# sjtuyinjie/Ground-Fusion2

Measured on AMD Instinct MI355X. Metric: sliding-window solves/sec (10-kf, 2k landmarks), higher is better.
Workload: dtype f64; 1 GPU; BASELINE configs[1]: 10-keyframe VI-wheel window, 2000 landmarks (K=9457 visual factors avg), marginalisation prior n=86, full optimization() = <=8 dogleg iterations + re-anchor + MARGIN_OLD; windows_per_gpu=8192, unique_windows=8, parallelism=windows sharded over 1 rank(s), no collective

## Files before the change

### ground-fusion2_amd/csrc/gfbe_devutil.h

```cpp
#pragma once
#include "gfbe_device.h"

namespace gfd {

#define GF_MIN_DIAG 1e-6
#define GF_MAX_DIAG 1e32
#define GF_MIN_MU 1e-8
#define GF_MAX_MU 1.0
#define GF_MU_INC 10.0

__device__ __forceinline__ double wave_sum(double v) {
#pragma unroll
  for (int o = 32; o > 0; o >>= 1) v += __shfl_down(v, o, 64);
  return v;
}
__device__ __forceinline__ double wave_max(double v) {
#pragma unroll
  for (int o = 32; o > 0; o >>= 1) v = fmax(v, __shfl_down(v, o, 64));
  return v;
}
__device__ __forceinline__ double block_sum(double v, double *scratch ) {
  v = wave_sum(v);
  const int lane = threadIdx.x & 63, wid = threadIdx.x >> 6;
  __syncthreads();
  if (lane == 0) scratch[wid] = v;
  __syncthreads();
  double r = 0.0;
  if (threadIdx.x == 0) for (int i = 0; i < (int)((blockDim.x + 63) >> 6); i++) r += scratch[i];
  return r;
}
__device__ __forceinline__ double block_max(double v, double *scratch) {
  v = wave_max(v);
  const int lane = threadIdx.x & 63, wid = threadIdx.x >> 6;
  __syncthreads();
  if (lane == 0) scratch[wid] = v;
  __syncthreads();
  double r = 0.0;
  if (threadIdx.x == 0) for (int i = 0; i < (int)((blockDim.x + 63) >> 6); i++) r = fmax(r, scratch[i]);
  return r;
}

template <int NQ>
__device__ __forceinline__ void block_reduce_multi(const double (&v)[NQ], unsigned maxmask, double *scratch, int tid = -1) {
  if (tid < 0) tid = threadIdx.x;
  const int lane = tid & 63, wid = tid >> 6, nw = (blockDim.x + 63) >> 6;
  __syncthreads();
#pragma unroll
  for (int q = 0; q < NQ; q++) {
    const double r = ((maxmask >> q) & 1) ? wave_max(v[q]) : wave_sum(v[q]);
    if (lane == 0) scratch[q * 16 + wid] = r;
  }
  __syncthreads();
  if (tid < NQ) {
// ... 43 lines not shown
```

### ground-fusion2_amd/csrc/gfbe_kernels.hip

```cpp
#include "gfbe_devutil.h"
#include "gfbe_factors.h"
#include "gfbe_gnss_item.h"
#include <type_traits>

namespace gfd {

#ifndef GFBE_ASM_U
#define GFBE_ASM_U 4
#endif
#if GFBE_DIAG
#define ASM_TP_ON(d) (!(d).asm_legacy)
#else
#define ASM_TP_ON(d) true
#endif
#ifndef GFBE_KVIS_WAVES
#define GFBE_KVIS_WAVES 3
#endif
#ifndef GFBE_KVIS_STAMP
#define GFBE_KVIS_STAMP 0
#endif

#define PREP_WSYNC() do { __threadfence_block(); __builtin_amdgcn_wave_barrier(); } while (0)
template <int n>
__device__ __forceinline__ int sqrt_info_from_cov_wave(const double *cov, double *lu, double *inv, double *U, const int lane) {
// ... 208 lines not shown
  const WinDesc &ds = d.desc[w];
  if (tile >= ds.n_tiles || !TILE_OWNED(d, tile)) return;
  const WinCtl &c = d.ctl[w];
  if (MODE == 0 && !SPEC && (c.done || c.reuse)) return;
  if (CAND && (c.done || !c.have_step)) return;
  int sframe = 0;
#pragma unroll
  for (int q = 1; q < NF; q++) sframe += (tile >= ds.sf_tile_begin[q]) ? 1 : 0;
  if (MODE == 2 && sframe != 0) return;
  const int buf = CAND ? 1 - c.cur : c.cur;
  const double *X = (MODE == 2) ? d.xout + (size_t)w * NA : d.x + ((size_t)w * 2 + buf) * NA;
  const double *lamv = d.lam + (size_t)buf * d.tot_lm;

#if GFBE_KVIS_STAMP
  double *kstamp = d.timing + (size_t)d.B * 32;
  const bool kst = MODE == 0 && w == d.B / 2 && tile == 0 && threadIdx.x == 0 && c.iter == 0;
#define KSTAMP(i) do { if (kst) kstamp[i] = (double)wall_clock64(); } while (0)
#else
#define KSTAMP(i) do { } while (0)
#endif
#if GFBE_LIN_STAMP
  unsigned long long *lst = (unsigned long long *)(d.timing + (size_t)d.B * 32);
  const bool lstamp = KS > 1 && MODE == 0 && tile == 0 && (threadIdx.x & 63) == 0 && (WS || threadIdx.x == 0);
#define LSTAMP(i) do { if (lstamp && kq == 0) lst[i] = wall_clock64(); } while (0)
#define LSTAMP_ANY(i) do { if (lstamp) lst[i] = wall_clock64(); } while (0)
#else
#define LSTAMP(i) do { } while (0)
#define LSTAMP_ANY(i) do { } while (0)
#endif
  LSTAMP(14);
  KSTAMP(0);
  constexpr bool YM = (MODE == 0 && !FULL);
  typedef typename std::conditional<FULL, PairConst, typename std::conditional<MODE == 2, PairConstR, PairConstY>::type>::type PCT;
  constexpr int PCW = (MODE == 1) ? 12 : sizeof(PCT) / sizeof(double), XLD = FULL ? XS_LD : 17;
  __shared__ PCT pcs[NF];
  __shared__ FrameConst fcs;
  __shared__ double xs_own[(MODE == 1 || WS) ? 1 : LM_TILE * XLD];
  double *const xs = WS ? wsm + (size_t)kq * (LM_TILE * XLD) : xs_own;
  const int lane = WS ? (threadIdx.x & 63) : threadIdx.x;
  const int slot = ds.lm_off + tile * LM_TILE + lane;
  const size_t TL = d.tot_lm;
  const bool tdc = YM || (MODE == 1 && !d.vis_full);
  const int nobq = tdc ? 2 : 5;
  const int info = d.lm_info[slot];
  const double pix = d.lm_pts[0 * TL + slot], piy = d.lm_pts[1 * TL + slot], piz = d.lm_pts[2 * TL + slot];
  double vix = 0.0, viy = 0.0, tdi = 0.0;
  if (!tdc) { vix = d.lm_pts[3 * TL + slot]; viy = d.lm_pts[4 * TL + slot]; tdi = d.lm_pts[5 * TL + slot]; }
  const bool chead = CAND && head;
  double lam = chead ? d.lam[(size_t)c.cur * TL + slot] : lamv[slot];
  double c_sl = 0.0, c_vl = 0.0, c_yl = 0.0;
  if (chead) { c_sl = d.lm_sl[slot]; c_vl = d.lm_vl[slot]; c_yl = d.lm_yl[slot]; }
  const double td = X[A_TD];
  double nob[5] = {0.0, 0.0, 0.0, 0.0, 0.0};
  {
    const double *ob = d.lm_obs + (size_t)kq * 5 * TL + slot;
#pragma unroll
    for (int q = 0; q < 5; q++) if (q < nobq) nob[q] = ob[q * TL];
  }
  constexpr int NLATER = KS > 1 ? (MAXOBS + KS - 1) / KS - 1 : 0;
  double nobl[NLATER > 0 ? NLATER : 1][5];
#pragma unroll
  for (int u = 0; u < NLATER; u++) {
#pragma unroll
    for (int q = 0; q < 5; q++) nobl[u][q] = 0.0;
    if (kq + (u + 1) * KS < MAXOBS) {
      const double *ob = d.lm_obs + (size_t)(kq + (u + 1) * KS) * 5 * TL + slot;
#pragma unroll
      for (int q = 0; q < 5; q++) if (q < nobq) nobl[u][q] = ob[q * TL];
    }
  }
// ... 33 lines not shown
  }
  if (chead) {
    double d2, n2;
    lam = candidate_lm(lam, c_sl, c_vl, c_yl, c.c1, c.c2, valid && !is_const && m > 0, d2, n2);
    d.lam[(size_t)(1 - c.cur) * TL + slot] = lam;
    d2 = wave_sum(d2); n2 = wave_sum(n2);
    if (lane == 0) {
      double *o = d.tile_cand + ((size_t)w * d.max_tiles + tile) * 4;
      o[1] = d2; o[2] = n2;
    }
  }

  constexpr int NHC = FULL ? HC : 6;
  double hC[NHC], Hll = 0.0, gl = 0.0;
#pragma unroll
  for (int q = 0; q < NHC; q++) hC[q] = 0.0;
  if (MODE != 1 && !FULL && !YM) {
    double *xr = xs + lane * XLD;
    xr[13] = 0.0; xr[14] = 0.0; xr[15] = 0.0;
  }
  double ycx = 0.0, ycy = 0.0, ycz = 0.0, yinv_l = 0.0, Dsum[3] = {0.0, 0.0, 0.0};
  vec3 yf = mk3(0.0, 0.0, 0.0), ye = yf, yx = yf;
  if (YM || MODE == 1) {
    const double dti = tdc ? 0.0 : td - tdi;
    yinv_l = 1.0 / lam;
    ycx = (tdc ? pix : __builtin_fma(-dti, vix, pix)) * yinv_l; ycy = (tdc ? piy : __builtin_fma(-dti, viy, piy)) * yinv_l; ycz = piz * yinv_l;
    if (YM) {
#pragma unroll
      for (int a = 0; a < 3; a++) {
        yf[a] = __builtin_fma(fcs.W(a, 0), ycx, __builtin_fma(fcs.W(a, 1), ycy, fcs.W(a, 2) * ycz));
        ye[a] = yf[a] + fcs.wt[a];
        yx[a] = ye[a] + fcs.dPc[a];
      }
      double *xr = xs + lane * XLD;
      xr[7] = 0.0; xr[15] = 0.0;
    }
  }
  KSTAMP(2);
  double *contrib = KS > 1 ? d.vis_contrib + (((size_t)w * d.max_tiles + tile) * MAXOBS) * (VC_STRIDE * LM_TILE) + lane : nullptr;
  for (int k = kq; k < mmax; k += KS) {
    if (k < 5) KSTAMP(3 + 5 * k);
    double r[2], Ji[12], Jj[12], Je[FULL ? 12 : 1], Jl[2], Jt[2], hp[6];
    const double pjx = nob[0], pjy = nob[1], vjx = nob[2], vjy = nob[3], tdj = nob[4];
    if (KS > 1) {
#pragma unroll
      for (int q = 0; q < 5; q++) nob[q] = nobl[0][q];
#pragma unroll
      for (int u = 0; u + 1 < NLATER; u++) {
#pragma unroll
        for (int q = 0; q < 5; q++) nobl[u][q] = nobl[u + 1][q];
      }
    } else if (k + KS < mmax) {
      const double *ob = d.lm_obs + (size_t)(k + KS) * 5 * TL + slot;
#pragma unroll
      for (int q = 0; q < 5; q++) if (q < nobq) nob[q] = ob[q * TL];
    }
    if constexpr (YM) {
      double *xr = xs + lane * XLD;
      if (k < m) {
        const PCT &pc = pcs[sframe + 1 + k];
        double g0[3], g1[3];
        const double ck = visual_lin_y(pc, ycx, ycy, ycz, yf, yinv_l, td, pjx, pjy, vjx, vjy, tdj, sq, delta, r, g0, g1, Jl);
        if (KS > 1) contrib[((size_t)k * VC_STRIDE + 15) * LM_TILE] = ck; else cost += ck;
        const vec3 y0 = cross3(mk3(g0[0], g0[1], g0[2]), yx), y1 = cross3(mk3(g1[0], g1[1], g1[2]), yx);
        const double w0 = is_const ? 0.0 : Jl[0], w1 = is_const ? 0.0 : Jl[1];
        vec3 dv;
#pragma unroll
        for (int q = 0; q < 3; q++) dv[q] = __builtin_fma(g0[q], w0, g1[q] * w1);
        if (KS > 1) {
          double *cb = contrib + (size_t)k * VC_STRIDE * LM_TILE;
          cb[0] = __builtin_fma(w0, w0, w1 * w1);
          cb[LM_TILE] = __builtin_fma(w0, r[0], w1 * r[1]);
#pragma unroll
          for (int q = 0; q < 3; q++) cb[(2 + q) * LM_TILE] = dv[q];
        } else {
          Hll += __builtin_fma(w0, w0, w1 * w1);
          gl += __builtin_fma(w0, r[0], w1 * r[1]);
#pragma unroll
          for (int q = 0; q < 3; q++) Dsum[q] += dv[q];
        }
#pragma unroll
        for (int q = 0; q < 3; q++) hp[q] = dv[q];
#pragma unroll
        for (int q = 0; q < 3; q++) { xr[q] = g0[q]; xr[3 + q] = y0[q]; xr[8 + q] = g1[q]; xr[11 + q] = y1[q]; }
        xr[6] = r[0]; xr[14] = r[1];
      } else {
#pragma unroll
        for (int q = 0; q < 7; q++) { xr[q] = 0.0; xr[8 + q] = 0.0; }
      }
#pragma unroll
      for (int q = 0; q < 2; q++) asm volatile("" : "+v"(nob[q]));
      if (k < m) {
#pragma unroll
        for (int q = 0; q < 3; q++) d.lm_hP[((size_t)k * 6 + q) * TL + slot] = hp[q];
      }
      typedef double dbl4_y __attribute__((ext_vector_type(4)));
      dbl4_y acc0 = {0, 0, 0, 0};
      const int lr = lane & 15, lk = lane >> 4;
      __threadfence_block();
      __builtin_amdgcn_wave_barrier();
#pragma unroll
      for (int blk = 0; blk < LM_TILE / 4 / 8; blk++) {
        double va[8];
#pragma unroll
        for (int u = 0; u < 8; u++) va[u] = xs[(4 * (8 * blk + u) + lk) * XLD + lr];
#pragma unroll
        for (int u = 0; u < 8; u++) acc0 = __builtin_amdgcn_mfma_f64_16x16x4f64(va[u], va[u], acc0, 0, 0, 0);
      }
      __builtin_amdgcn_wave_barrier();
      const double s0 = acc0[0] + __shfl_down(acc0[2], 8, 64), s1 = acc0[1] + __shfl_down(acc0[3], 8, 64);
      double *vo = d.vis_part + (((size_t)w * d.max_tiles + tile) * MAXOBS + k) * VPY_STRIDE;
      if (lr < 7) {
        { const int a = lk; if (a <= lr) vo[7 * a - a * (a - 1) / 2 + lr - a] = s0; }
        { const int a = lk + 4; if (a <= lr) vo[7 * a - a * (a - 1) / 2 + lr - a] = s1; }
      }
      __builtin_amdgcn_wave_barrier();
    }
    if constexpr (MODE == 1) {
      if (k < m) cost += visual_cost_y(pcs[sframe + 1 + k], ycx, ycy, ycz, td, pjx, pjy, vjx, vjy, tdj, sq, delta);
    }
    if constexpr (!YM && MODE != 1) {
    if (k < m) {
      const double ck = visual_lin<MODE != 1, FULL>(pcs[sframe + 1 + k], lam, td, pix, piy, piz, pjx, pjy, vix, viy, vjx, vjy, tdi, tdj,
                                                    sq, delta, r, Ji, Jj, Je, Jl, Jt);
      if (KS > 1) contrib[((size_t)k * VC_STRIDE + 15) * LM_TILE] = ck; else cost += ck;
      if (MODE != 1) {
        if (FULL && write_records) {
          double *rb = d.rec + ((size_t)ds.rec_off + d.lm_rec[(size_t)k * TL + slot]) * REC;
          rb[0] = r[0]; rb[1] = r[1];
#pragma unroll
          for (int q = 0; q < 6; q++) {
            rb[2 + q] = Ji[q]; rb[8 + q] = Jj[q]; rb[14 + q] = Je[FULL ? q : 0];
            rb[22 + q] = Ji[6 + q]; rb[28 + q] = Jj[6 + q]; rb[34 + q] = Je[FULL ? 6 + q : 0];
          }
          rb[20] = Jl[0]; rb[21] = Jt[0]; rb[40] = Jl[1]; rb[41] = Jt[1];
        }
        const double w0 = (is_const && MODE == 0) ? 0.0 : Jl[0], w1 = (is_const && MODE == 0) ? 0.0 : Jl[1];
        if (KS > 1) {
          double *cb = contrib + (size_t)k * VC_STRIDE * LM_TILE;
          cb[0] = __builtin_fma(w0, w0, w1 * w1);
          cb[LM_TILE] = __builtin_fma(w0, r[0], w1 * r[1]);
#pragma unroll
          for (int q = 0; q < 6; q++) {
            cb[(2 + q) * LM_TILE] = __builtin_fma(Ji[q], w0, Ji[6 + q] * w1);
            if (FULL) cb[(8 + q) * LM_TILE] = __builtin_fma(Je[q], w0, Je[6 + q] * w1);
            hp[q] = __builtin_fma(Jj[q], w0, Jj[6 + q] * w1);
          }
          if (FULL) cb[14 * LM_TILE] = __builtin_fma(Jt[0], w0, Jt[1] * w1);
        } else {
// ... 182 lines not shown
}

__device__ __forceinline__ double candidate_tile(const BatchDev &d, const WinDesc &ds, const WinCtl &c, const int w, const int tile, const int t);
template <int MODE, bool FULL, bool SPEC = false>
__global__ __launch_bounds__(LM_TILE, (MODE == 0 && !FULL) ? GFBE_KVIS_WAVES : 2) void k_vis(BatchDev d0, int write_records) {
  const BatchDev d = MODE == 0 ? lin_view(d0, SPEC ? 1 - d0.ctl[blockIdx.x].lb : d0.ctl[blockIdx.x].lb) : d0;
  vis_body<MODE, FULL, 1, SPEC>(d, (MODE == 1 || SPEC) ? 0 : write_records, blockIdx.x, blockIdx.y, 0, (MODE == 1 || SPEC) && write_records);
}

#ifndef VIS_CHUNK
#define VIS_CHUNK 4
#endif
template <bool SPEC>
__global__ __launch_bounds__(LM_TILE, GFBE_KVIS_WAVES) void k_vis_chunk(BatchDev d0, int head_in, int nsub) {
  const int w = blockIdx.x;
  const WinCtl &c = d0.ctl[w];
  if (!SPEC && (c.done || c.reuse)) return;
  if (SPEC && (c.done || !c.have_step)) return;
  const int lbw = SPEC ? 1 - c.lb : c.lb;
  const BatchDev d = lin_view(d0, lbw);
  const WinDesc &ds = d.desc[w];
  const int sframe = blockIdx.y / nsub, sub = blockIdx.y - sframe * nsub;
  const int t0 = ds.sf_tile_begin[sframe] + VIS_CHUNK * sub, t1 = min(t0 + VIS_CHUNK, ds.sf_tile_begin[sframe + 1]);
  if (t0 >= t1) return;
  const int cur = c.cur, buf = SPEC ? 1 - cur : cur;
  const double *X = d.x + ((size_t)w * 2 + buf) * NA;
  const bool chead = SPEC && head_in;
  const double c1 = c.c1, c2 = c.c2;
  const bool first = !SPEC && c.iter == 0;
  const double mu_w = SPEC ? mu_after_accept(c.mu) : c.mu;
  const double sq = d.opt.vis_sqrt_info, delta = d.opt.huber_delta;
  const int jac_scale = d.opt.jacobi_scaling;
  const int lm_off_c = ds.lm_off;
  constexpr int XLD = 17;
  __shared__ PairConstY pcs[NF];
  __shared__ FrameConst fcs;
  __shared__ double xs[LM_TILE * XLD];
  const int lane = threadIdx.x;
  const size_t TL = d.tot_lm;
  int p_info;
  double p_pt[3], p_lam, p_sl = 0.0, p_vl = 0.0, p_yl = 0.0, p_ob[2];
#define VC_PREFETCH(TILE)                                                                                           \
  {                                                                                                                  \
    const int slot_ = lm_off_c + (TILE) * LM_TILE + lane;                                                            \
    p_info = d.lm_info[slot_];                                                                                       \
    _Pragma("unroll") for (int q = 0; q < 3; q++) p_pt[q] = d.lm_pts[(size_t)q * TL + slot_];                        \
    p_lam = d.lam[(size_t)(chead ? cur : buf) * TL + slot_];                                                         \
    if (chead) { p_sl = d.lm_sl[slot_]; p_vl = d.lm_vl[slot_]; p_yl = d.lm_yl[slot_]; }                              \
    p_ob[0] = d.lm_obs[slot_]; p_ob[1] = d.lm_obs[TL + slot_];                                                       \
  }
  VC_PREFETCH(t0)
  const double td = X[A_TD];
  {
    const double *src = d.pc + (((size_t)w * 3 + buf) * NPAIR + sframe * NF) * PC_DOUBLES;
    static_assert(PCY_DOUBLES <= LM_TILE && FC_DOUBLES <= LM_TILE, "one lane per entry of a pair record");
    const int ql = min(lane, (int)PCY_DOUBLES - 1);
    double rec[NF - 1];
#pragma unroll
    for (int jj = 0; jj < NF - 1; jj++) rec[jj] = src[(size_t)min(sframe + 1 + jj, NF - 1) * PC_DOUBLES + ql];
    const double fcv = src[(size_t)sframe * PC_DOUBLES + min(lane, (int)FC_DOUBLES - 1)];
#pragma unroll
    for (int jj = 0; jj < NF - 1; jj++) if (sframe + 1 + jj < NF && lane < (int)PCY_DOUBLES) ((double *)&pcs[min(sframe + 1 + jj, NF - 1)])[lane] = rec[jj];
    if (lane < (int)FC_DOUBLES) ((double *)&fcs)[lane] = fcv;
  }
  __syncthreads();
  for (int tile = t0; tile < t1; tile++) {
    const int slot = lm_off_c + tile * LM_TILE + lane;
    const int info = p_info;
    const double pix = p_pt[0], piy = p_pt[1], piz = p_pt[2];
    double lam = p_lam;
    const double c_sl = p_sl, c_vl = p_vl, c_yl = p_yl;
    double nob[2] = {p_ob[0], p_ob[1]};
    if (tile + 1 < t1) VC_PREFETCH(tile + 1)
    const bool valid = (info >> 24) & 1;
    const int m = valid ? ((info >> 8) & 0xff) : 0;
    const bool is_const = (info >> 16) & 1;
    int mmax = m;
#pragma unroll
    for (int o = 32; o > 0; o >>= 1) mmax = max(mmax, __shfl_xor(mmax, o, 64));
    double cost = 0.0;
    if (chead) {
      double d2, n2;
      lam = candidate_lm(lam, c_sl, c_vl, c_yl, c1, c2, valid && !is_const && m > 0, d2, n2);
      d.lam[(size_t)(1 - cur) * TL + slot] = lam;
      d2 = wave_sum(d2); n2 = wave_sum(n2);
      if (lane == 0) {
        double *o = d.tile_cand + ((size_t)w * d.max_tiles + tile) * 4;
        o[1] = d2; o[2] = n2;
      }
    }
    double Hll = 0.0, gl = 0.0, Dsum[3] = {0.0, 0.0, 0.0};
    const double yinv_l = 1.0 / lam;
    const double ycx = pix * yinv_l, ycy = piy * yinv_l, ycz = piz * yinv_l;
    vec3 yf, ye, yx;
#pragma unroll
    for (int a = 0; a < 3; a++) {
      yf[a] = __builtin_fma(fcs.W(a, 0), ycx, __builtin_fma(fcs.W(a, 1), ycy, fcs.W(a, 2) * ycz));
      ye[a] = yf[a] + fcs.wt[a];
      yx[a] = ye[a] + fcs.dPc[a];
    }
    double *xr = xs + lane * XLD;
    xr[7] = 0.0; xr[15] = 0.0;
    for (int k = 0; k < mmax; k++) {
      double r[2], Jl[2], hp[3];
      const double pjx = nob[0], pjy = nob[1];
      if (k + 1 < mmax) {
        const double *ob = d.lm_obs + (size_t)(k + 1) * 5 * TL + slot;
        nob[0] = ob[0]; nob[1] = ob[TL];
      }
      if (k < m) {
        double g0[3], g1[3];
        const double ck = visual_lin_y(pcs[sframe + 1 + k], ycx, ycy, ycz, yf, yinv_l, td, pjx, pjy, 0.0, 0.0, td, sq, delta, r, g0, g1, Jl);
        cost += ck;
        const vec3 y0 = cross3(mk3(g0[0], g0[1], g0[2]), yx), y1 = cross3(mk3(g1[0], g1[1], g1[2]), yx);
        const double w0 = is_const ? 0.0 : Jl[0], w1 = is_const ? 0.0 : Jl[1];
        vec3 dv;
#pragma unroll
        for (int q = 0; q < 3; q++) dv[q] = __builtin_fma(g0[q], w0, g1[q] * w1);
        Hll += __builtin_fma(w0, w0, w1 * w1);
        gl += __builtin_fma(w0, r[0], w1 * r[1]);
#pragma unroll
        for (int q = 0; q < 3; q++) Dsum[q] += dv[q];
#pragma unroll
        for (int q = 0; q < 3; q++) hp[q] = dv[q];
#pragma unroll
        for (int q = 0; q < 3; q++) { xr[q] = g0[q]; xr[3 + q] = y0[q]; xr[8 + q] = g1[q]; xr[11 + q] = y1[q]; }
        xr[6] = r[0]; xr[14] = r[1];
      } else {
#pragma unroll
        for (int q = 0; q < 7; q++) { xr[q] = 0.0; xr[8 + q] = 0.0; }
      }
#pragma unroll
      for (int q = 0; q < 2; q++) asm volatile("" : "+v"(nob[q]));
      if (k < m) {
#pragma unroll
        for (int q = 0; q < 3; q++) d.lm_hP[((size_t)k * 6 + q) * TL + slot] = hp[q];
      }
      typedef double dbl4_y __attribute__((ext_vector_type(4)));
      dbl4_y acc0 = {0, 0, 0, 0};
      const int lr = lane & 15, lk = lane >> 4;
      __threadfence_block();
      __builtin_amdgcn_wave_barrier();
#pragma unroll
      for (int blk = 0; blk < LM_TILE / 4 / 8; blk++) {
        double va[8];
#pragma unroll
        for (int u = 0; u < 8; u++) va[u] = xs[(4 * (8 * blk + u) + lk) * XLD + lr];
#pragma unroll
        for (int u = 0; u < 8; u++) acc0 = __builtin_amdgcn_mfma_f64_16x16x4f64(va[u], va[u], acc0, 0, 0, 0);
      }
      __builtin_amdgcn_wave_barrier();
      const double s0 = acc0[0] + __shfl_down(acc0[2], 8, 64), s1 = acc0[1] + __shfl_down(acc0[3], 8, 64);
      double *vo = d.vis_part + (((size_t)w * d.max_tiles + tile) * MAXOBS + k) * VPY_STRIDE;
      if (lr < 7) {
        { const int a = lk; if (a <= lr) vo[7 * a - a * (a - 1) / 2 + lr - a] = s0; }
        { const int a = lk + 4; if (a <= lr) vo[7 * a - a * (a - 1) / 2 + lr - a] = s1; }
      }
      __builtin_amdgcn_wave_barrier();
    }
    if (d.spec && tile == 0 && lane == 0) d.ctl[w].sw_mu[lbw] = mu_w;
    if (valid) {
      double sl = 1.0, sw = 0.0;
      if (m > 0 && !is_const) {
        sl = first ? (jac_scale ? 1.0 / (1.0 + sqrt(Hll)) : 1.0) : (chead ? c_sl : d.lm_sl[slot]);
        const double hs2 = sl * sl * Hll;
        sw = sqrt(sl * sl / (hs2 + mu_w * clamp_diag(hs2)));
      }
      if (first) d.lm_sl[slot] = sl;
      d.lm_sw[slot] = sw;
      d.lm_Hll[slot] = Hll;
      d.lm_gl[slot] = gl;
#pragma unroll
      for (int q = 0; q < 3; q++) { d.lm_hC[(size_t)q * TL + slot] = Dsum[q]; d.lm_hC[(size_t)(3 + q) * TL + slot] = yx[q]; }
    }
    cost = wave_sum(cost);
    if (lane == 0) {
      if (SPEC) d.tile_cand[((size_t)w * d.max_tiles + tile) * 4] = cost;
      else d.tile_cost[(size_t)w * d.max_tiles + tile] = cost;
    }
  }
#undef VC_PREFETCH
}

template <int MODE, bool FULL>
__global__ __launch_bounds__(LM_TILE, 1) void k_vis_split(BatchDev d, int write_records) {
  vis_body<MODE, FULL, LIN_SMALL_KS>(d, write_records, blockIdx.x, blockIdx.y / LIN_SMALL_KS, blockIdx.y % LIN_SMALL_KS);
}

template <int MODE>
__global__ __launch_bounds__(256) void k_lio_window(BatchDev d0, int spec) {
  const int w = blockIdx.y, wg = blockIdx.x, t = threadIdx.x;
// ... 782 lines not shown
    SCHUR_SLOT(3, acc3)                                                                                                  \
  }
  double preA[SCHUR_PV], aHll = 0.0, aSl = 0.0;
  int aInfo = 0, aS = 0;
  SCHUR_PREFETCH(preA, aHll, aSl, aInfo, aS, tfirst)
  for (int tile = tfirst; tile < te; tile += tstep) SCHUR_RUN_TILE(preA, aHll, aSl, aInfo, aS, tile, tile + tstep)
#undef SCHUR_RUN_TILE
#undef SCHUR_SLOT
#undef SCHUR_PREFETCH
#undef SCHUR_PV
  if (stamp_wg) { stamp[3] = (double)wall_clock64(); stamp[4] = (double)(te - tb); stamp[6] = (double)clock64(); }
  double *out = d.schur_part + ((size_t)w * d.schur_groups + grp) * SCHUR_STRIDE;
#define SCHUR_OUT(Q, ACC)                                                         \
  if (pI[Q] >= 0) {                                                               \
    double *o = out + (size_t)(compact ? pJ[Q] * (pJ[Q] + 1) / 2 + pI[Q] : schur_pair(pI[Q], pJ[Q])) * 256; \
    _Pragma("unroll") for (int r = 0; r < 4; r++) o[(lk + 4 * r) * 16 + lr] = ACC[r]; \
  }
  SCHUR_OUT(0, acc0)
  SCHUR_OUT(1, acc1)
  SCHUR_OUT(2, acc2)
  SCHUR_OUT(3, acc3)
#undef SCHUR_OUT
}
#ifndef GFBE_SCHUR_WGS
#define GFBE_SCHUR_WGS 4
#endif
__global__ __launch_bounds__(256, GFBE_SCHUR_WGS) void k_schur(BatchDev d0, int marg) {
  const BatchDev d = marg ? d0 : lin_view(d0, d0.ctl[blockIdx.x].lb);
  schur_body(d, marg, blockIdx.x, blockIdx.y);
}
#ifndef GFBE_LINSCHUR_WGS
#define GFBE_LINSCHUR_WGS 3
#endif
#define LS_XLD 17
template <bool SPEC>
__global__ __launch_bounds__(256, GFBE_LINSCHUR_WGS) void k_linschur(BatchDev d0, int head_in, int gate_mu) {
  const int w = blockIdx.x;
  const int grp = blockIdx.y == 1 ? 2 : (blockIdx.y == 2 ? 1 : (int)blockIdx.y);
  const WinCtl &c = d0.ctl[w];
  if (c.done) return;
  if (SPEC) { if (!c.have_step) return; }
  else { if (c.reuse) return; if (gate_mu && c.sw_mu[c.lb] == c.mu) return; }
  const int lbw = SPEC ? 1 - c.lb : c.lb;
  const BatchDev d = lin_view(d0, lbw);
  const WinDesc &ds = d.desc[w];
  const int s_first = schur_group_first(grp, SCHUR_GROUPS), s_end = grp == SCHUR_GROUPS - 1 ? (int)NF : schur_group_first(grp + 1, SCHUR_GROUPS);
  const int tb = ds.sf_tile_begin[s_first], te = ds.sf_tile_begin[s_end];
  if (tb >= te) return;
  __shared__ double hs[LM_TILE * HS_LD + 8];
  static_assert(4 * LM_TILE * LS_XLD <= LM_TILE * HS_LD + 8, "the evaluation panels live inside the Schur panel");
  __shared__ double Psum[4][5][LM_TILE];
  __shared__ double Pcost[4];
  __shared__ PairConstY pcs[NF];
  __shared__ FrameConst fcs;
  __shared__ double s_rt[NF][12];
  const int t = threadIdx.x, lane = t & 63, wave = t >> 6;
  const int wv = __builtin_amdgcn_readfirstlane(wave);
  const int rot = __builtin_amdgcn_readfirstlane((int)(((unsigned)w * 0x9E3779B1u) >> 20) + grp);
  const int mr = (wv + rot) & 3;
  const size_t TL = d.tot_lm;
  const int cur = c.cur;
  const int buf = SPEC ? 1 - cur : cur;
  const double *X = d.x + ((size_t)w * 2 + buf) * NA;
  const double *pcw = d.pc + ((size_t)w * 3 + buf) * NPAIR * PC_DOUBLES;
  const bool chead = SPEC && head_in;
  const double c1 = c.c1, c2 = c.c2;
  const bool first = !SPEC && c.iter == 0;
  const double mu_w = SPEC ? mu_after_accept(c.mu) : c.mu;
  const double sq = d.opt.vis_sqrt_info, delta = d.opt.huber_delta;
  const int jac_scale = d.opt.jacobi_scaling;
  const double td = X[A_TD];
  int sfb[NF + 1];
#pragma unroll
  for (int q = 0; q <= NF; q++) sfb[q] = ds.sf_tile_begin[q];
  const int lm_off_c = ds.lm_off;
  if (t < NF * 12) s_rt[t / 12][t % 12] = pcw[(size_t)(t / 12) * (NF + 1) * PC_DOUBLES + LM_RT_OFF + t % 12];
  const int coff = 1 - 6 * s_first;
  const int nside = (1 + 6 * (NF - s_first) + 15) / 16, npairs = nside * (nside + 1) / 2;
  int pI[4], pJ[4];
#pragma unroll
  for (int q = 0; q < 4; q++) {
    const int idx = 4 * q + mr;
    pI[q] = -1; pJ[q] = -1;
    if (idx < npairs) { int J = 0; while ((J + 1) * (J + 2) / 2 <= idx) J++; pJ[q] = J; pI[q] = idx - J * (J + 1) / 2; }
  }
  dbl4_t acc0 = {0.0, 0.0, 0.0, 0.0}, acc1 = acc0, acc2 = acc0, acc3 = acc0;
  const int lr = lane & 15, lk = lane >> 4;
  double *const xs = hs + (size_t)wave * (LM_TILE * LS_XLD);
  int p_info;
  double p_pt[3], p_lam, p_sl = 1.0, p_vl = 0.0, p_yl = 0.0, p_ob[3][2];
#define LS_PREFETCH(TILE)                                                                                           \
  {                                                                                                                  \
    const int er_ = (wv + rot + (TILE)) & 3;                                                                         \
    const int tile_ = min((TILE), te - 1);                                                                           \
    const int slot_ = lm_off_c + tile_ * LM_TILE + lane;                                                             \
    p_info = d.lm_info[slot_];                                                                                       \
    _Pragma("unroll") for (int q = 0; q < 3; q++) p_pt[q] = d.lm_pts[(size_t)q * TL + slot_];                        \
    p_lam = d.lam[(size_t)(chead ? cur : buf) * TL + slot_];                                                         \
    if (chead) { p_vl = d.lm_vl[slot_]; p_yl = d.lm_yl[slot_]; }                                                     \
    if (!first) p_sl = d.lm_sl[slot_];                                                                               \
    _Pragma("unroll") for (int u = 0; u < 3; u++) {                                                                  \
      const int k_ = min(er_ + 4 * u, (int)MAXOBS - 1);                                                              \
      p_ob[u][0] = d.lm_obs[((size_t)k_ * 5 + 0) * TL + slot_];                                                      \
      p_ob[u][1] = d.lm_obs[((size_t)k_ * 5 + 1) * TL + slot_];                                                      \
    }                                                                                                                \
  }
  LS_PREFETCH(tb)
  int cur_sf = -1;
  for (int tile = tb; tile < te; tile++) {
    int sf = s_first;
#pragma unroll
    for (int q = 1; q < NF; q++) sf += (q > s_first && q < s_end && tile >= sfb[q]) ? 1 : 0;
    if (sf != cur_sf) {
      const double *src = pcw + (size_t)sf * NF * PC_DOUBLES;
      for (int e = t; e < (NF - 1 - sf) * (int)PCY_DOUBLES; e += 256) {
        const int j = sf + 1 + e / (int)PCY_DOUBLES, q = e % (int)PCY_DOUBLES;
        ((double *)&pcs[j])[q] = src[(size_t)j * PC_DOUBLES + q];
      }
      if (t < (int)FC_DOUBLES) ((double *)&fcs)[t] = src[(size_t)sf * PC_DOUBLES + t];
      cur_sf = sf;
    }
    __syncthreads();
    const int er = (wv + rot + tile) & 3;
    const int slot = lm_off_c + tile * LM_TILE + lane;
    const int info = p_info;
    const bool valid = (info >> 24) & 1;
    const int m = valid ? ((info >> 8) & 0xff) : 0;
    const bool is_const = (info >> 16) & 1;
    int mmax = m;
#pragma unroll
    for (int o = 32; o > 0; o >>= 1) mmax = max(mmax, __shfl_xor(mmax, o, 64));
    mmax = __builtin_amdgcn_readfirstlane(mmax);
    double lam = p_lam;
    const double sl_old = p_sl;
    if (chead) {
      double d2, n2;
      lam = candidate_lm(lam, sl_old, p_vl, p_yl, c1, c2, valid && !is_const && m > 0, d2, n2);
      if (er == 0) {
        d.lam[(size_t)(1 - cur) * TL + slot] = lam;
        d2 = wave_sum(d2); n2 = wave_sum(n2);
        if (lane == 0) { double *o = d.tile_cand + ((size_t)w * d.max_tiles + tile) * 4; o[1] = d2; o[2] = n2; }
      }
    }
    const double yinv_l = 1.0 / lam;
    const double ycx = p_pt[0] * yinv_l, ycy = p_pt[1] * yinv_l, ycz = p_pt[2] * yinv_l;
    vec3 yf, yx;
#pragma unroll
    for (int a = 0; a < 3; a++) {
      yf[a] = __builtin_fma(fcs.W(a, 0), ycx, __builtin_fma(fcs.W(a, 1), ycy, fcs.W(a, 2) * ycz));
      yx[a] = (yf[a] + fcs.wt[a]) + fcs.dPc[a];
    }
    double *xr = xs + lane * LS_XLD;
    xr[7] = 0.0; xr[15] = 0.0;
    double Hq = 0.0, gq = 0.0, Dq[3] = {0.0, 0.0, 0.0}, cq = 0.0, dk[3][3];
#pragma unroll
    for (int u = 0; u < 3; u++) {
      dk[u][0] = 0.0; dk[u][1] = 0.0; dk[u][2] = 0.0;
      const int k = er + 4 * u;
      if (k < mmax) {
        if (k < m) {
          double r[2], g0[3], g1[3], Jl[2];
          cq += visual_lin_y(pcs[sf + 1 + k], ycx, ycy, ycz, yf, yinv_l, td, p_ob[u][0], p_ob[u][1], 0.0, 0.0, td, sq, delta, r, g0, g1, Jl);
          const vec3 y0 = cross3(mk3(g0[0], g0[1], g0[2]), yx), y1 = cross3(mk3(g1[0], g1[1], g1[2]), yx);
          const double w0 = is_const ? 0.0 : Jl[0], w1 = is_const ? 0.0 : Jl[1];
#pragma unroll
          for (int q = 0; q < 3; q++) dk[u][q] = __builtin_fma(g0[q], w0, g1[q] * w1);
          Hq += __builtin_fma(w0, w0, w1 * w1);
          gq += __builtin_fma(w0, r[0], w1 * r[1]);
#pragma unroll
          for (int q = 0; q < 3; q++) Dq[q] += dk[u][q];
#pragma unroll
          for (int q = 0; q < 3; q++) { xr[q] = g0[q]; xr[3 + q] = y0[q]; xr[8 + q] = g1[q]; xr[11 + q] = y1[q]; }
          xr[6] = r[0]; xr[14] = r[1];
#pragma unroll
          for (int q = 0; q < 3; q++) d.lm_hP[((size_t)k * 6 + q) * TL + slot] = dk[u][q];
        } else {
#pragma unroll
          for (int q = 0; q < 7; q++) { xr[q] = 0.0; xr[8 + q] = 0.0; }
        }
        dbl4_t a0 = {0, 0, 0, 0};
        __threadfence_block();
        __builtin_amdgcn_wave_barrier();
#pragma unroll
        for (int blk = 0; blk < LM_TILE / 4 / 8; blk++) {
          double va[8];
#pragma unroll
          for (int v = 0; v < 8; v++) va[v] = xs[(4 * (8 * blk + v) + lk) * LS_XLD + lr];
#pragma unroll
          for (int v = 0; v < 8; v++) a0 = __builtin_amdgcn_mfma_f64_16x16x4f64(va[v], va[v], a0, 0, 0, 0);
        }
        __builtin_amdgcn_wave_barrier();
        const double s0 = a0[0] + __shfl_down(a0[2], 8, 64), s1 = a0[1] + __shfl_down(a0[3], 8, 64);
        double *vo = d.vis_part + (((size_t)w * d.max_tiles + tile) * MAXOBS + k) * VPY_STRIDE;
        if (lr < 7) {
          { const int a = lk; if (a <= lr) vo[7 * a - a * (a - 1) / 2 + lr - a] = s0; }
          { const int a = lk + 4; if (a <= lr) vo[7 * a - a * (a - 1) / 2 + lr - a] = s1; }
        }
        __builtin_amdgcn_wave_barrier();
      }
    }
    Psum[er][0][lane] = Hq; Psum[er][1][lane] = gq;
#pragma unroll
    for (int q = 0; q < 3; q++) Psum[er][2 + q][lane] = Dq[q];
    cq = wave_sum(cq);
    if (lane == 0) Pcost[er] = cq;
    __syncthreads();
    double Hll, gl, Dv[3];
    Hll = ((Psum[0][0][lane] + Psum[1][0][lane]) + Psum[2][0][lane]) + Psum[3][0][lane];
    gl = ((Psum[0][1][lane] + Psum[1][1][lane]) + Psum[2][1][lane]) + Psum[3][1][lane];
#pragma unroll
    for (int q = 0; q < 3; q++) Dv[q] = ((Psum[0][2 + q][lane] + Psum[1][2 + q][lane]) + Psum[2][2 + q][lane]) + Psum[3][2 + q][lane];
    double sl = 1.0, sw = 0.0;
    if (valid && m > 0 && !is_const) {
      sl = first ? (jac_scale ? 1.0 / (1.0 + sqrt(Hll)) : 1.0) : sl_old;
      const double hs2 = sl * sl * Hll;
      sw = sqrt(sl * sl / (hs2 + mu_w * clamp_diag(hs2)));
    }
    if (er == 2) {
      if (valid) {
        if (first) d.lm_sl[slot] = sl;
        d.lm_sw[slot] = sw;
        d.lm_Hll[slot] = Hll;
        d.lm_gl[slot] = gl;
#pragma unroll
        for (int q = 0; q < 3; q++) { d.lm_hC[(size_t)q * TL + slot] = Dv[q]; d.lm_hC[(size_t)(3 + q) * TL + slot] = yx[q]; }
      }
      if (lane == 0) {
        const double cost = ((Pcost[0] + Pcost[1]) + Pcost[2]) + Pcost[3];
        if (SPEC) d.tile_cand[((size_t)w * d.max_tiles + tile) * 4] = cost;
        else d.tile_cost[(size_t)w * d.max_tiles + tile] = cost;
        if (SPEC && d.spec && tile == 0) d.ctl[w].sw_mu[lbw] = mu_w;
// ... 1710 lines not shown
  hipLaunchKernelGGL(k_gather, dim3(GATHER_WGS, d.B), dim3(256), 0, s, d, margin_flag);
}
void launch_prep(const BatchDev &d, hipStream_t s) {
  hipLaunchKernelGGL(k_prep, dim3(d.B, PREP_FACT_WGS), dim3(256), 0, s, d);
  hipLaunchKernelGGL(k_prep_prior, dim3(d.B, PREP_PRIOR_WGS), dim3(256), 0, s, d);
}
void launch_reset(const BatchDev &d, hipStream_t s) {
  const int slots = d.max_tiles * LM_TILE;
  hipLaunchKernelGGL(k_reset, dim3((slots + 255) / 256 > 0 ? (slots + 255) / 256 : 1, d.B), dim3(256), 0, s, d);
}
void launch_vis(const BatchDev &d, int mode, hipStream_t s, int write_records, int spec) {
  if (d.max_tiles == 0) return;
  const dim3 g(d.B, d.max_tiles), b(LM_TILE);
  if (mode == 0 && !d.vis_full && !write_records && d.B >= DENSE_SPLIT_MIN_B && d.world == 1) {
    const int nsub = (d.max_sf_tiles + VIS_CHUNK - 1) / VIS_CHUNK;
    const dim3 gc(d.B, NF * nsub);
    if (spec) hipLaunchKernelGGL(k_vis_chunk<true>, gc, b, 0, s, d, 1, nsub);
    else hipLaunchKernelGGL(k_vis_chunk<false>, gc, b, 0, s, d, 0, nsub);
    return;
  }
  if (mode == 0 && spec) {
    const int head = d.B >= DENSE_SPLIT_MIN_B ? 1 : 0;
    if (d.vis_full) hipLaunchKernelGGL((k_vis<0, true, true>), g, b, 0, s, d, head);
    else hipLaunchKernelGGL((k_vis<0, false, true>), g, b, 0, s, d, head);
    return;
  }
  if (mode == 0 && (d.vis_full || write_records)) hipLaunchKernelGGL((k_vis<0, true>), g, b, 0, s, d, write_records);
  else if (mode == 0) hipLaunchKernelGGL((k_vis<0, false>), g, b, 0, s, d, 0);
  else if (mode == 1) hipLaunchKernelGGL((k_vis<1, true>), g, b, 0, s, d, d.B >= DENSE_SPLIT_MIN_B ? 1 : 0);
  else if (d.B < DENSE_SPLIT_MIN_B) hipLaunchKernelGGL((k_vis_split<2, true>), dim3(d.B, d.max_tiles * LIN_SMALL_KS), b, 0, s, d, write_records);
  else hipLaunchKernelGGL((k_vis<2, true>), g, b, 0, s, d, write_records);
}
static size_t lin_small_lds(bool split, bool full) {
  const size_t panels = split ? (size_t)LIN_SMALL_KS * LM_TILE * (full ? (size_t)XS_LD : 17) : 0;
  return sizeof(double) * std::max(panels, (size_t)PRIOR_CHUNK);
}
bool lin_small_takes_gnss(const BatchDev &d, int mode) { return d.any_gnss && (mode == 1 || mode == 3) && d.gnss_max_obs <= (int)GN_ITEM_MAX_OBS; }
void launch_lin_small(const BatchDev &d, int mode, hipStream_t s, int fuse) {
  const dim3 g(d.B, d.max_tiles + MAX_IMU + MAX_WHEEL + 1 + (d.any_plane ? MAX_PLANE + 1 : 0) + (lin_small_takes_gnss(d, mode) ? 1 : 0)), b(LIN_SMALL_THREADS);
  if (mode == 2) hipLaunchKernelGGL((k_lin_small<2, true>), g, b, lin_small_lds(true, true), s, d, 0);
  else if (mode == 0 && d.vis_full) hipLaunchKernelGGL((k_lin_small<0, true>), g, b, lin_small_lds(true, true), s, d, 0);
  else if (mode == 0) hipLaunchKernelGGL((k_lin_small<0, false>), g, b, lin_small_lds(true, false), s, d, 0);
  else if (mode == 3 && d.vis_full) hipLaunchKernelGGL((k_lin_small<3, true>), g, b, lin_small_lds(true, true), s, d, fuse);
  else if (mode == 3) hipLaunchKernelGGL((k_lin_small<3, false>), g, b, lin_small_lds(true, false), s, d, fuse);
  else hipLaunchKernelGGL((k_lin_small<1, true>), g, b, lin_small_lds(false, true), s, d, fuse);
}
hipError_t lin_small_init_device() {
  hipError_t e = hipSuccess;
  auto set = [&](const void *k, size_t bytes) { if (e == hipSuccess) e = hipFuncSetAttribute(k, hipFuncAttributeMaxDynamicSharedMemorySize, (int)bytes); };
  set((const void *)k_lin_small<2, true>, lin_small_lds(true, true));
  set((const void *)k_lin_small<0, true>, lin_small_lds(true, true));
  set((const void *)k_lin_small<0, false>, lin_small_lds(true, false));
  set((const void *)k_lin_small<3, true>, lin_small_lds(true, true));
  set((const void *)k_lin_small<3, false>, lin_small_lds(true, false));
  set((const void *)k_lin_small<1, true>, lin_small_lds(false, true));
  return e;
}
void launch_pair_schur_marg(const BatchDev &d, hipStream_t s) {
  if (d.max_tiles == 0) { launch_pair(d, 1, s); return; }
  hipLaunchKernelGGL(k_pairsum_schur_marg, dim3(d.B, NF), dim3(VP_STRIDE), 0, s, d);
}
void launch_pair(const BatchDev &d, int marg, hipStream_t s) {
  hipLaunchKernelGGL(k_pairsum, dim3(marg ? NF - 1 : NF * (NF - 1) / 2, d.B), dim3(VP_STRIDE), 0, s, d, marg);
}
void launch_dense_factors(const BatchDev &d, int mode, int debug_out, hipStream_t s, int spec) {
  const int nf = MAX_IMU + MAX_WHEEL + 1 + (d.any_plane ? MAX_PLANE + 1 : 0);
  if (d.B < DENSE_SPLIT_MIN_B) {
// ... 84 lines not shown
```

Baseline: 125,900 solves/s.

## Use 4x4x4 f64 MFMA with swizzled 16-wide panels for visual Gram blocks

Replaces the per-observation 7x7 Gram accumulation, previously a padded 17-stride panel fed to 16x16x4 f64 MFMA, with a 16-stride XOR-swizzled panel written as double2 chunks and reduced with 4x4x4 f64 MFMAs plus DPP row folds. The aim is to cut wasted MFMA work on padding, avoid LDS bank conflicts through the swizzle, use vectorized LDS stores, and shrink the LDS panel footprint. The new layout and index mapping is intricate, so a wrong mapping would silently corrupt the Hessian blocks.

```diff
diff --git a/ground-fusion2_amd/csrc/gfbe_devutil.h b/ground-fusion2_amd/csrc/gfbe_devutil.h
--- a/ground-fusion2_amd/csrc/gfbe_devutil.h
+++ b/ground-fusion2_amd/csrc/gfbe_devutil.h
@@ -19,6 +19,52 @@
   for (int o = 32; o > 0; o >>= 1) v = fmax(v, __shfl_down(v, o, 64));
   return v;
 }
+#define VG_LD 16
+typedef double dbl2_vg __attribute__((ext_vector_type(2)));
+__device__ __forceinline__ dbl2_vg *vis_gram_chunk(double *xs, const int f, const int h, const int lj) {
+  return (dbl2_vg *)(xs + f * VG_LD + 2 * ((4 * h + lj) ^ (f & 7)));
+}
+__device__ __forceinline__ void vis_gram_row(double *xs, const int f, const int h, const double g[3], const double y0, const double y1, const double y2,
+                                             const double r) {
+  *vis_gram_chunk(xs, f, h, 0) = dbl2_vg{g[0], y1};
+  *vis_gram_chunk(xs, f, h, 1) = dbl2_vg{g[1], y2};
+  *vis_gram_chunk(xs, f, h, 2) = dbl2_vg{g[2], r};
+  *vis_gram_chunk(xs, f, h, 3) = dbl2_vg{y0, 0.0};
+}
+__device__ __forceinline__ void vis_gram_zero(double *xs, const int f) {
+#pragma unroll
+  for (int c = 0; c < 8; c++) ((dbl2_vg *)(xs + f * VG_LD))[c] = dbl2_vg{0.0, 0.0};
+}
+template <int CTRL>
+__device__ __forceinline__ double vis_gram_fold(const double x) {
+  const int lo = __builtin_amdgcn_update_dpp(0, __double2loint(x), CTRL, 0xf, 0xf, false);
+  const int hi = __builtin_amdgcn_update_dpp(0, __double2hiint(x), CTRL, 0xf, 0xf, false);
+  return x + __hiloint2double(hi, lo);
+}
+__device__ __forceinline__ void vis_gram_store(double *xs, const int lane, double *vo) {
+  const int lk = lane >> 4, lb = (lane >> 2) & 3, lj = lane & 3;
+  double a00 = 0.0, a01 = 0.0, a11 = 0.0;
+  __threadfence_block();
+  __builtin_amdgcn_wave_barrier();
+  dbl2_vg v[8];
+#pragma unroll
+  for (int u = 0; u < 8; u++) v[u] = *vis_gram_chunk(xs, 16 * (u & 3) + 4 * lb + lk, u >> 2, lj);
+#pragma unroll
+  for (int u = 0; u < 8; u++) {
+    a00 = __builtin_amdgcn_mfma_f64_4x4x4f64(v[u].x, v[u].x, a00, 0, 0, 0);
+    a01 = __builtin_amdgcn_mfma_f64_4x4x4f64(v[u].x, v[u].y, a01, 0, 0, 0);
+    a11 = __builtin_amdgcn_mfma_f64_4x4x4f64(v[u].y, v[u].y, a11, 0, 0, 0);
+  }
+  __builtin_amdgcn_wave_barrier();
+  a00 = vis_gram_fold<0x128>(vis_gram_fold<0x124>(a00));
+  a01 = vis_gram_fold<0x128>(vis_gram_fold<0x124>(a01));
+  a11 = vis_gram_fold<0x128>(vis_gram_fold<0x124>(a11));
+  const int a = lk + (lb == 2 ? 4 : 0), b = lj + (lb >= 1 ? 4 : 0);
+  const double s = lb == 0 ? a00 : (lb == 1 ? a01 : a11);
+  if (lb < 3 && a <= b && b < 7) vo[7 * a - a * (a - 1) / 2 + b - a] = s;
+  __builtin_amdgcn_wave_barrier();
+}
+
 __device__ __forceinline__ double block_sum(double v, double *scratch ) {
   v = wave_sum(v);
   const int lane = threadIdx.x & 63, wid = threadIdx.x >> 6;
diff --git a/ground-fusion2_amd/csrc/gfbe_kernels.hip b/ground-fusion2_amd/csrc/gfbe_kernels.hip
--- a/ground-fusion2_amd/csrc/gfbe_kernels.hip
+++ b/ground-fusion2_amd/csrc/gfbe_kernels.hip
@@ -264,10 +264,10 @@
   KSTAMP(0);
   constexpr bool YM = (MODE == 0 && !FULL);
   typedef typename std::conditional<FULL, PairConst, typename std::conditional<MODE == 2, PairConstR, PairConstY>::type>::type PCT;
-  constexpr int PCW = (MODE == 1) ? 12 : sizeof(PCT) / sizeof(double), XLD = FULL ? XS_LD : 17;
+  constexpr int PCW = (MODE == 1) ? 12 : sizeof(PCT) / sizeof(double), XLD = FULL ? XS_LD : (MODE == 0 ? VG_LD : 17);
   __shared__ PCT pcs[NF];
   __shared__ FrameConst fcs;
-  __shared__ double xs_own[(MODE == 1 || WS) ? 1 : LM_TILE * XLD];
+  __shared__ __attribute__((aligned(16))) double xs_own[(MODE == 1 || WS) ? 1 : LM_TILE * XLD];
   double *const xs = WS ? wsm + (size_t)kq * (LM_TILE * XLD) : xs_own;
   const int lane = WS ? (threadIdx.x & 63) : threadIdx.x;
   const int slot = ds.lm_off + tile * LM_TILE + lane;
@@ -367,8 +367,6 @@
         ye[a] = yf[a] + fcs.wt[a];
         yx[a] = ye[a] + fcs.dPc[a];
       }
-      double *xr = xs + lane * XLD;
-      xr[7] = 0.0; xr[15] = 0.0;
     }
   }
   KSTAMP(2);
@@ -391,7 +389,6 @@
       for (int q = 0; q < 5; q++) if (q < nobq) nob[q] = ob[q * TL];
     }
     if constexpr (YM) {
-      double *xr = xs + lane * XLD;
       if (k < m) {
         const PCT &pc = pcs[sframe + 1 + k];
         double g0[3], g1[3];
@@ -416,12 +413,10 @@
         }
 #pragma unroll
         for (int q = 0; q < 3; q++) hp[q] = dv[q];
-#pragma unroll
-        for (int q = 0; q < 3; q++) { xr[q] = g0[q]; xr[3 + q] = y0[q]; xr[8 + q] = g1[q]; xr[11 + q] = y1[q]; }
-        xr[6] = r[0]; xr[14] = r[1];
+        vis_gram_row(xs, lane, 0, g0, y0[0], y0[1], y0[2], r[0]);
+        vis_gram_row(xs, lane, 1, g1, y1[0], y1[1], y1[2], r[1]);
       } else {
-#pragma unroll
-        for (int q = 0; q < 7; q++) { xr[q] = 0.0; xr[8 + q] = 0.0; }
+        vis_gram_zero(xs, lane);
       }
 #pragma unroll
       for (int q = 0; q < 2; q++) asm volatile("" : "+v"(nob[q]));
@@ -429,27 +424,7 @@
 #pragma unroll
         for (int q = 0; q < 3; q++) d.lm_hP[((size_t)k * 6 + q) * TL + slot] = hp[q];
       }
-      typedef double dbl4_y __attribute__((ext_vector_type(4)));
-      dbl4_y acc0 = {0, 0, 0, 0};
-      const int lr = lane & 15, lk = lane >> 4;
-      __threadfence_block();
-      __builtin_amdgcn_wave_barrier();
-#pragma unroll
-      for (int blk = 0; blk < LM_TILE / 4 / 8; blk++) {
-        double va[8];
-#pragma unroll
-        for (int u = 0; u < 8; u++) va[u] = xs[(4 * (8 * blk + u) + lk) * XLD + lr];
-#pragma unroll
-        for (int u = 0; u < 8; u++) acc0 = __builtin_amdgcn_mfma_f64_16x16x4f64(va[u], va[u], acc0, 0, 0, 0);
-      }
-      __builtin_amdgcn_wave_barrier();
-      const double s0 = acc0[0] + __shfl_down(acc0[2], 8, 64), s1 = acc0[1] + __shfl_down(acc0[3], 8, 64);
-      double *vo = d.vis_part + (((size_t)w * d.max_tiles + tile) * MAXOBS + k) * VPY_STRIDE;
-      if (lr < 7) {
-        { const int a = lk; if (a <= lr) vo[7 * a - a * (a - 1) / 2 + lr - a] = s0; }
-        { const int a = lk + 4; if (a <= lr) vo[7 * a - a * (a - 1) / 2 + lr - a] = s1; }
-      }
-      __builtin_amdgcn_wave_barrier();
+      vis_gram_store(xs, lane, d.vis_part + (((size_t)w * d.max_tiles + tile) * MAXOBS + k) * VPY_STRIDE);
     }
     if constexpr (MODE == 1) {
       if (k < m) cost += visual_cost_y(pcs[sframe + 1 + k], ycx, ycy, ycz, td, pjx, pjy, vjx, vjy, tdj, sq, delta);
@@ -698,10 +673,9 @@
   const double sq = d.opt.vis_sqrt_info, delta = d.opt.huber_delta;
   const int jac_scale = d.opt.jacobi_scaling;
   const int lm_off_c = ds.lm_off;
-  constexpr int XLD = 17;
   __shared__ PairConstY pcs[NF];
   __shared__ FrameConst fcs;
-  __shared__ double xs[LM_TILE * XLD];
+  __shared__ __attribute__((aligned(16))) double xs[LM_TILE * VG_LD];
   const int lane = threadIdx.x;
   const size_t TL = d.tot_lm;
   int p_info;
@@ -765,8 +739,6 @@
       ye[a] = yf[a] + fcs.wt[a];
       yx[a] = ye[a] + fcs.dPc[a];
     }
-    double *xr = xs + lane * XLD;
-    xr[7] = 0.0; xr[15] = 0.0;
     for (int k = 0; k < mmax; k++) {
       double r[2], Jl[2], hp[3];
       const double pjx = nob[0], pjy = nob[1];
@@ -789,12 +761,10 @@
         for (int q = 0; q < 3; q++) Dsum[q] += dv[q];
 #pragma unroll
         for (int q = 0; q < 3; q++) hp[q] = dv[q];
-#pragma unroll
-        for (int q = 0; q < 3; q++) { xr[q] = g0[q]; xr[3 + q] = y0[q]; xr[8 + q] = g1[q]; xr[11 + q] = y1[q]; }
-        xr[6] = r[0]; xr[14] = r[1];
+        vis_gram_row(xs, lane, 0, g0, y0[0], y0[1], y0[2], r[0]);
+        vis_gram_row(xs, lane, 1, g1, y1[0], y1[1], y1[2], r[1]);
       } else {
-#pragma unroll
-        for (int q = 0; q < 7; q++) { xr[q] = 0.0; xr[8 + q] = 0.0; }
+        vis_gram_zero(xs, lane);
       }
 #pragma unroll
       for (int q = 0; q < 2; q++) asm volatile("" : "+v"(nob[q]));
@@ -802,27 +772,7 @@
 #pragma unroll
         for (int q = 0; q < 3; q++) d.lm_hP[((size_t)k * 6 + q) * TL + slot] = hp[q];
       }
-      typedef double dbl4_y __attribute__((ext_vector_type(4)));
-      dbl4_y acc0 = {0, 0, 0, 0};
-      const int lr = lane & 15, lk = lane >> 4;
-      __threadfence_block();
-      __builtin_amdgcn_wave_barrier();
-#pragma unroll
-      for (int blk = 0; blk < LM_TILE / 4 / 8; blk++) {
-        double va[8];
-#pragma unroll
-        for (int u = 0; u < 8; u++) va[u] = xs[(4 * (8 * blk + u) + lk) * XLD + lr];
-#pragma unroll
-        for (int u = 0; u < 8; u++) acc0 = __builtin_amdgcn_mfma_f64_16x16x4f64(va[u], va[u], acc0, 0, 0, 0);
-      }
-      __builtin_amdgcn_wave_barrier();
-      const double s0 = acc0[0] + __shfl_down(acc0[2], 8, 64), s1 = acc0[1] + __shfl_down(acc0[3], 8, 64);
-      double *vo = d.vis_part + (((size_t)w * d.max_tiles + tile) * MAXOBS + k) * VPY_STRIDE;
-      if (lr < 7) {
-        { const int a = lk; if (a <= lr) vo[7 * a - a * (a - 1) / 2 + lr - a] = s0; }
-        { const int a = lk + 4; if (a <= lr) vo[7 * a - a * (a - 1) / 2 + lr - a] = s1; }
-      }
-      __builtin_amdgcn_wave_barrier();
+      vis_gram_store(xs, lane, d.vis_part + (((size_t)w * d.max_tiles + tile) * MAXOBS + k) * VPY_STRIDE);
     }
     if (d.spec && tile == 0 && lane == 0) d.ctl[w].sw_mu[lbw] = mu_w;
     if (valid) {
@@ -1671,7 +1621,6 @@
 #ifndef GFBE_LINSCHUR_WGS
 #define GFBE_LINSCHUR_WGS 3
 #endif
-#define LS_XLD 17
 template <bool SPEC>
 __global__ __launch_bounds__(256, GFBE_LINSCHUR_WGS) void k_linschur(BatchDev d0, int head_in, int gate_mu) {
   const int w = blockIdx.x;
@@ -1686,8 +1635,8 @@
   const int s_first = schur_group_first(grp, SCHUR_GROUPS), s_end = grp == SCHUR_GROUPS - 1 ? (int)NF : schur_group_first(grp + 1, SCHUR_GROUPS);
   const int tb = ds.sf_tile_begin[s_first], te = ds.sf_tile_begin[s_end];
   if (tb >= te) return;
-  __shared__ double hs[LM_TILE * HS_LD + 8];
-  static_assert(4 * LM_TILE * LS_XLD <= LM_TILE * HS_LD + 8, "the evaluation panels live inside the Schur panel");
+  __shared__ __attribute__((aligned(16))) double hs[LM_TILE * HS_LD + 8];
+  static_assert(4 * LM_TILE * VG_LD <= LM_TILE * HS_LD + 8, "the evaluation panels live inside the Schur panel");
   __shared__ double Psum[4][5][LM_TILE];
   __shared__ double Pcost[4];
   __shared__ PairConstY pcs[NF];
@@ -1725,7 +1674,7 @@
   }
   dbl4_t acc0 = {0.0, 0.0, 0.0, 0.0}, acc1 = acc0, acc2 = acc0, acc3 = acc0;
   const int lr = lane & 15, lk = lane >> 4;
-  double *const xs = hs + (size_t)wave * (LM_TILE * LS_XLD);
+  double *const xs = hs + (size_t)wave * (LM_TILE * VG_LD);
   int p_info;
   double p_pt[3], p_lam, p_sl = 1.0, p_vl = 0.0, p_yl = 0.0, p_ob[3][2];
 #define LS_PREFETCH(TILE)                                                                                           \
@@ -1789,8 +1738,6 @@
       yf[a] = __builtin_fma(fcs.W(a, 0), ycx, __builtin_fma(fcs.W(a, 1), ycy, fcs.W(a, 2) * ycz));
       yx[a] = (yf[a] + fcs.wt[a]) + fcs.dPc[a];
     }
-    double *xr = xs + lane * LS_XLD;
-    xr[7] = 0.0; xr[15] = 0.0;
     double Hq = 0.0, gq = 0.0, Dq[3] = {0.0, 0.0, 0.0}, cq = 0.0, dk[3][3];
 #pragma unroll
     for (int u = 0; u < 3; u++) {
@@ -1808,34 +1755,14 @@
           gq += __builtin_fma(w0, r[0], w1 * r[1]);
 #pragma unroll
           for (int q = 0; q < 3; q++) Dq[q] += dk[u][q];
-#pragma unroll
-          for (int q = 0; q < 3; q++) { xr[q] = g0[q]; xr[3 + q] = y0[q]; xr[8 + q] = g1[q]; xr[11 + q] = y1[q]; }
-          xr[6] = r[0]; xr[14] = r[1];
+          vis_gram_row(xs, lane, 0, g0, y0[0], y0[1], y0[2], r[0]);
+          vis_gram_row(xs, lane, 1, g1, y1[0], y1[1], y1[2], r[1]);
 #pragma unroll
           for (int q = 0; q < 3; q++) d.lm_hP[((size_t)k * 6 + q) * TL + slot] = dk[u][q];
         } else {
-#pragma unroll
-          for (int q = 0; q < 7; q++) { xr[q] = 0.0; xr[8 + q] = 0.0; }
+          vis_gram_zero(xs, lane);
         }
-        dbl4_t a0 = {0, 0, 0, 0};
-        __threadfence_block();
-        __builtin_amdgcn_wave_barrier();
-#pragma unroll
-        for (int blk = 0; blk < LM_TILE / 4 / 8; blk++) {
-          double va[8];
-#pragma unroll
-          for (int v = 0; v < 8; v++) va[v] = xs[(4 * (8 * blk + v) + lk) * LS_XLD + lr];
-#pragma unroll
-          for (int v = 0; v < 8; v++) a0 = __builtin_amdgcn_mfma_f64_16x16x4f64(va[v], va[v], a0, 0, 0, 0);
-        }
-        __builtin_amdgcn_wave_barrier();
-        const double s0 = a0[0] + __shfl_down(a0[2], 8, 64), s1 = a0[1] + __shfl_down(a0[3], 8, 64);
-        double *vo = d.vis_part + (((size_t)w * d.max_tiles + tile) * MAXOBS + k) * VPY_STRIDE;
-        if (lr < 7) {
-          { const int a = lk; if (a <= lr) vo[7 * a - a * (a - 1) / 2 + lr - a] = s0; }
-          { const int a = lk + 4; if (a <= lr) vo[7 * a - a * (a - 1) / 2 + lr - a] = s1; }
-        }
-        __builtin_amdgcn_wave_barrier();
+        vis_gram_store(xs, lane, d.vis_part + (((size_t)w * d.max_tiles + tile) * MAXOBS + k) * VPY_STRIDE);
       }
     }
     Psum[er][0][lane] = Hq; Psum[er][1][lane] = gq;
@@ -3612,7 +3539,7 @@
   else hipLaunchKernelGGL((k_vis<2, true>), g, b, 0, s, d, write_records);
 }
 static size_t lin_small_lds(bool split, bool full) {
-  const size_t panels = split ? (size_t)LIN_SMALL_KS * LM_TILE * (full ? (size_t)XS_LD : 17) : 0;
+  const size_t panels = split ? (size_t)LIN_SMALL_KS * LM_TILE * (full ? (size_t)XS_LD : (size_t)VG_LD) : 0;
   return sizeof(double) * std::max(panels, (size_t)PRIOR_CHUNK);
 }
 bool lin_small_takes_gnss(const BatchDev &d, int mode) { return d.any_gnss && (mode == 1 || mode == 3) && d.gnss_max_obs <= (int)GN_ITEM_MAX_OBS; }
```

New measurement: 124,400 solves/s. 1.2% lower.
